# computations/root_digger

Hardware: NVIDIA B200
Metric: root_placements_per_sec (higher is better)
Workload: dtype f64

## Files before the change

### root_digger_b200/csrc/rdk_kernels.cuh

```cuda
#pragma once
#include <cuda_runtime.h>
#include "rdk_lower.hpp"
#include <stdint.h>
#include <type_traits>

namespace rdk {

constexpr int kMaxCats = 32;

__device__ __forceinline__ double dmul(double a, double b) { return __dmul_rn(a, b); }
__device__ __forceinline__ double dadd(double a, double b) { return __dadd_rn(a, b); }
__device__ __forceinline__ double dsub(double a, double b) { return __dsub_rn(a, b); }
__device__ __forceinline__ double ddiv(double a, double b) { return __ddiv_rn(a, b); }
__device__ __forceinline__ double dfma(double a, double b, double c) { return __fma_rn(a, b, c); }

#define RDK_SCALE_THRESHOLD 0x1p-256
#define RDK_SCALE_FACTOR 0x1p+256
#define RDK_LOG_SCALE_THRESHOLD (-177.44567822334599)

static __constant__ double kLogConst[9] = {
    6.93147180369123816490e-01, 1.90821492927058770002e-10,
    6.666666666666735130e-01,   3.999999999940941908e-01,
    2.857142874366239149e-01,   2.222219843214978396e-01,
    1.818357216161805012e-01,   1.531383769920937332e-01,
// ... 53 lines not shown
    }
}

__device__ __forceinline__ double norm1_4(const double* A) {
  double best = 0.0;
#pragma unroll
  for (int j = 0; j < 4; ++j) {
    double s = fabs(A[0 * 4 + j]);
    s = dadd(s, fabs(A[1 * 4 + j]));
    s = dadd(s, fabs(A[2 * 4 + j]));
    s = dadd(s, fabs(A[3 * 4 + j]));
    if (s > best) best = s;
  }
  return best;
}

__device__ inline void solve4(double* M, double* N, double* X) {
  for (int c = 0; c < 4; ++c) {
    int    piv = c;
    double best = fabs(M[c * 4 + c]);
    for (int r = c + 1; r < 4; ++r) {
      double v = fabs(M[r * 4 + c]);
      if (v > best) {
        best = v;
        piv = r;
      }
    }
    if (piv != c) {
      for (int j = 0; j < 4; ++j) {
        double t = M[c * 4 + j];
        M[c * 4 + j] = M[piv * 4 + j];
        M[piv * 4 + j] = t;
        t = N[c * 4 + j];
        N[c * 4 + j] = N[piv * 4 + j];
        N[piv * 4 + j] = t;
      }
    }
    for (int r = c + 1; r < 4; ++r) {
      double f = ddiv(M[r * 4 + c], M[c * 4 + c]);
      for (int j = c + 1; j < 4; ++j) M[r * 4 + j] = dsub(M[r * 4 + j], dmul(f, M[c * 4 + j]));
      for (int j = 0; j < 4; ++j) N[r * 4 + j] = dsub(N[r * 4 + j], dmul(f, N[c * 4 + j]));
    }
  }
  for (int r = 3; r >= 0; --r)
    for (int j = 0; j < 4; ++j) {
      double s = N[r * 4 + j];
      for (int q = r + 1; q < 4; ++q) s = dsub(s, dmul(M[r * 4 + q], X[q * 4 + j]));
      X[r * 4 + j] = ddiv(s, M[r * 4 + r]);
    }
}

__device__ inline void expm4(const double* Ain, double* E) {
  const double TH3 = 1.495585217958292e-2, TH5 = 2.539398330063230e-1,
               TH7 = 9.504178996162932e-1, TH9 = 2.097847961257068e0,
               TH13 = 5.371920351148152e0;
  double A[16], U[16], V[16];
#pragma unroll
  for (int i = 0; i < 16; ++i) A[i] = Ain[i];
  double n1 = norm1_4(A);
  int    s = 0;
  int    deg = 13;
  if (n1 <= TH3)
    deg = 3;
  else if (n1 <= TH5)
    deg = 5;
  else if (n1 <= TH7)
    deg = 7;
  else if (n1 <= TH9)
    deg = 9;
  if (deg == 13) {
    while (n1 > TH13) {
      n1 = dmul(n1, 0.5);
      ++s;
    }
    double sc = __longlong_as_double((long long)(uint64_t)(1023 - s) << 52);
#pragma unroll
    for (int i = 0; i < 16; ++i) A[i] = dmul(A[i], sc);
  }
  double A2[16], A4[16], A6[16];
  mm4(A, A, A2);
  if (deg == 13) {
    const double b0 = 64764752532480000., b1 = 32382376266240000., b2 = 7771770303897600.,
                 b3 = 1187353796428800., b4 = 129060195264000., b5 = 10559470521600.,
                 b6 = 670442572800., b7 = 33522128640., b8 = 1323241920., b9 = 40840800.,
                 b10 = 960960., b11 = 16380., b12 = 182., b13 = 1.;
    double W1[16], Z1[16], W[16], T[16];
    mm4(A2, A2, A4);
    mm4(A4, A2, A6);
#pragma unroll
    for (int i = 0; i < 16; ++i) {
      double t = dmul(b13, A6[i]);
      t = dadd(t, dmul(b11, A4[i]));
      t = dadd(t, dmul(b9, A2[i]));
      W1[i] = t;
      t = dmul(b12, A6[i]);
      t = dadd(t, dmul(b10, A4[i]));
      t = dadd(t, dmul(b8, A2[i]));
      Z1[i] = t;
    }
    mm4(A6, W1, T);
#pragma unroll
    for (int i = 0; i < 16; ++i) {
      double id = (i % 5 == 0) ? 1.0 : 0.0;
      double t = dmul(b7, A6[i]);
      t = dadd(t, dmul(b5, A4[i]));
      t = dadd(t, dmul(b3, A2[i]));
      t = dadd(t, dmul(b1, id));
      W[i] = dadd(T[i], t);
    }
    mm4(A, W, U);
    mm4(A6, Z1, T);
#pragma unroll
    for (int i = 0; i < 16; ++i) {
      double id = (i % 5 == 0) ? 1.0 : 0.0;
      double t = dmul(b6, A6[i]);
      t = dadd(t, dmul(b4, A4[i]));
      t = dadd(t, dmul(b2, A2[i]));
      t = dadd(t, dmul(b0, id));
      V[i] = dadd(T[i], t);
    }
  } else {
    double A8[16], W[16];
    if (deg >= 5) mm4(A2, A2, A4);
    if (deg >= 7) mm4(A4, A2, A6);
    if (deg >= 9) mm4(A6, A2, A8);
    for (int i = 0; i < 16; ++i) {
      double id = (i % 5 == 0) ? 1.0 : 0.0;
      double w, v;
      if (deg == 3) {
        w = dmul(1., A2[i]);
        v = dmul(12., A2[i]);
        W[i] = dadd(w, dmul(60., id));
        V[i] = dadd(v, dmul(120., id));
      } else if (deg == 5) {
        w = dmul(1., A4[i]);
        w = dadd(w, dmul(420., A2[i]));
        v = dmul(30., A4[i]);
        v = dadd(v, dmul(3360., A2[i]));
        W[i] = dadd(w, dmul(15120., id));
        V[i] = dadd(v, dmul(30240., id));
      } else if (deg == 7) {
        w = dmul(1., A6[i]);
        w = dadd(w, dmul(1512., A4[i]));
        w = dadd(w, dmul(277200., A2[i]));
        v = dmul(56., A6[i]);
        v = dadd(v, dmul(25200., A4[i]));
        v = dadd(v, dmul(1995840., A2[i]));
        W[i] = dadd(w, dmul(8648640., id));
        V[i] = dadd(v, dmul(17297280., id));
      } else {
        w = dmul(1., A8[i]);
        w = dadd(w, dmul(3960., A6[i]));
        w = dadd(w, dmul(2162160., A4[i]));
        w = dadd(w, dmul(302702400., A2[i]));
        v = dmul(90., A8[i]);
        v = dadd(v, dmul(110880., A6[i]));
        v = dadd(v, dmul(30270240., A4[i]));
        v = dadd(v, dmul(2075673600., A2[i]));
        W[i] = dadd(w, dmul(8821612800., id));
        V[i] = dadd(v, dmul(17643225600., id));
      }
    }
    mm4(A, W, U);
  }
  double M[16], N[16];
#pragma unroll
  for (int i = 0; i < 16; ++i) {
    M[i] = dsub(V[i], U[i]);
    N[i] = dadd(V[i], U[i]);
  }
  solve4(M, N, E);
  for (int q = 0; q < s; ++q) {
    double T[16];
    mm4(E, E, T);
#pragma unroll
    for (int i = 0; i < 16; ++i) E[i] = T[i];
  }
}

__device__ inline void build_q_nonrev(const double* r, const double* pi, double* Q) {
  int k = 0;
  for (int i = 0; i < 4; ++i)
    for (int j = 0; j < 4; ++j)
      if (i != j) Q[i * 4 + j] = dmul(r[k++], pi[j]);
  for (int i = 0; i < 4; ++i) {
    double s = 0.0;
    bool   first = true;
    for (int j = 0; j < 4; ++j) {
      if (j == i) continue;
      if (first) {
        s = Q[i * 4 + j];
        first = false;
      } else
        s = dadd(s, Q[i * 4 + j]);
    }
    Q[i * 4 + i] = -s;
  }
  double mu = dmul(pi[0], -Q[0]);
  mu = dadd(mu, dmul(pi[1], -Q[5]));
  mu = dadd(mu, dmul(pi[2], -Q[10]));
  mu = dadd(mu, dmul(pi[3], -Q[15]));
  for (int i = 0; i < 16; ++i) Q[i] = ddiv(Q[i], mu);
}

__host__ __device__ __forceinline__ unsigned tip_mask_of_code(unsigned code) {
  return (unsigned)((0x0FEDCBA976538421ULL >> (4 * code)) & 15ULL);
}
__host__ __device__ __forceinline__ unsigned tip_code_of_mask(unsigned mask) {
  return (unsigned)((0xEDCBA9837652410FULL >> (4 * mask)) & 15ULL);
}

constexpr int kPTabDoubles = 18;
constexpr int kTipTabDoubles = 64;
constexpr int kTabDoubles = 64;
constexpr int kSlotDoubles = kPTabDoubles + kTipTabDoubles;

struct PmatEntry {
  unsigned slot;
  unsigned pad;
  double   t;
};

constexpr int kPmatInline = 16;
struct PmatArgs {
  const PmatEntry* entries;
  int              n;
  int              K;
  double           r[12];
  double           pi[4];
  double           pinv;
  double           rates[kMaxCats];
  double*          pool;
  PmatEntry        inl[kPmatInline];
};

#ifndef RDK_PROGRAM_KERNEL_ONLY
__global__ void __launch_bounds__(64) pmat_expm_nonrev_kernel(const __grid_constant__ PmatArgs a) {
  int tid = blockIdx.x * blockDim.x + threadIdx.x;
  if (tid >= a.n * a.K) return;
  int       e = tid / a.K, k = tid - e * a.K;
  PmatEntry ent = (a.n <= kPmatInline) ? a.inl[e] : a.entries[e];
  double    Q[16], A[16], E[16];
  double    r[12], pi[4];
  for (int i = 0; i < 12; ++i) r[i] = a.r[i];
  for (int i = 0; i < 4; ++i) pi[i] = a.pi[i];
  build_q_nonrev(r, pi, Q);
  double c = ddiv(dmul(a.rates[k], ent.t), dsub(1.0, a.pinv));
  for (int i = 0; i < 16; ++i) A[i] = dmul(Q[i], c);
  expm4(A, E);
  double* slot = a.pool + (size_t)ent.slot * a.K * kSlotDoubles;
  double* out = slot + (size_t)k * kPTabDoubles;
  for (int i = 0; i < 16; ++i) out[i] = E[i];
  out[16] = out[17] = 0.0;
  double* tab = slot + (size_t)a.K * kPTabDoubles;
  for (int i = 0; i < 4; ++i)
    for (unsigned code = 0; code < 16; ++code) {
      unsigned m = tip_mask_of_code(code);
      double   x = dmul(E[i * 4 + 0], (m & 1u) ? 1.0 : 0.0);
      x = dadd(x, dmul(E[i * 4 + 1], (m & 2u) ? 1.0 : 0.0));
      x = dadd(x, dmul(E[i * 4 + 2], (m & 4u) ? 1.0 : 0.0));
      x = dadd(x, dmul(E[i * 4 + 3], (m & 8u) ? 1.0 : 0.0));
      tab[((size_t)code * a.K + k) * 4 + i] = x;
    }
}

#endif

struct alignas(16) Instr {
  double*              parent;
  const void*          c1;
  const void*          c2;
  unsigned*            pscale;
  const unsigned*      c1scale;
  const unsigned*      c2scale;
  const double*        P1;
  const double*        P2;
  unsigned             flags;
  unsigned             slot;
  unsigned             pad[2];
};
static_assert(sizeof(Instr) == 80, "Instr layout");

constexpr int kProgInline = 8;
constexpr int kMaxChunks = 16;
struct ProgArgs {
  const Instr*    prog;
  int             n_instr;
  unsigned        nelem;
  unsigned        n_witer;
  unsigned        it0;
  const unsigned* weights;
  double*         partials;
  unsigned        partial_stride;
  double*         persite;
  unsigned        persite_unweighted;
  double          pi[4];
  double          w[kMaxCats];
  unsigned        n_chunks;
  unsigned        chunk_off[kMaxChunks + 1];
  Instr           inl[kProgInline];
  size_t          row_stride;
};

template <int K>
struct Ring {
  static constexpr int      kDepth = K <= 8 ? 8 : (K == 16 ? 4 : 2);
  static constexpr int      kLogDepth = kDepth == 8 ? 3 : (kDepth == 4 ? 2 : 1);
  static constexpr unsigned kTabBytes = kTabDoubles * K * 8;
  static constexpr unsigned kPBytes = kPTabDoubles * K * 8;
  static constexpr unsigned kInstrBytes = 128;
  static constexpr unsigned kSlotBytes = kInstrBytes + 2 * kTabBytes;
  static constexpr unsigned kSmemBytes = kDepth * kSlotBytes + 2 * kDepth * 8;
};

struct d4 {
  double v[4];
};

__device__ __forceinline__ d4 ld_clv(const void* base, unsigned e) {
  const char* q = reinterpret_cast<const char*>(base) + (size_t)e * 32u;
  d4          r;
  asm volatile("ld.global.cg.v4.f64 {%0,%1,%2,%3}, [%4];\n"
               : "=d"(r.v[0]), "=d"(r.v[1]), "=d"(r.v[2]), "=d"(r.v[3])
               : "l"(q));
  return r;
}
__device__ __forceinline__ void st_clv(double* base, unsigned e, const d4& x) {
  char* q = reinterpret_cast<char*>(base) + (size_t)e * 32u;
  asm volatile("st.global.cg.v4.f64 [%0], {%1,%2,%3,%4};\n" ::"l"(q), "d"(x.v[0]), "d"(x.v[1]), "d"(x.v[2]),
               "d"(x.v[3])
               : "memory");
}

__device__ __forceinline__ unsigned smem_u32(const void* p) { return (unsigned)__cvta_generic_to_shared(p); }
__device__ __forceinline__ void mbar_init(unsigned long long* bar, unsigned count) {
  asm volatile("mbarrier.init.shared::cta.b64 [%0], %1;\n" ::"r"(smem_u32(bar)), "r"(count) : "memory");
}
__device__ __forceinline__ void mbar_expect_tx(unsigned long long* bar, unsigned bytes) {
  asm volatile("mbarrier.arrive.expect_tx.shared::cta.b64 _, [%0], %1;\n" ::"r"(smem_u32(bar)), "r"(bytes)
               : "memory");
}
__device__ __forceinline__ void mbar_arrive(unsigned long long* bar) {
  asm volatile("mbarrier.arrive.shared::cta.b64 _, [%0];\n" ::"r"(smem_u32(bar)) : "memory");
}
__device__ __forceinline__ void mbar_wait(unsigned long long* bar, unsigned parity) {
  asm volatile(
      "{\n"
      ".reg .pred P1;\n"
      "LAB_WAIT:\n"
      "mbarrier.try_wait.parity.shared::cta.b64 P1, [%0], %1;\n"
      "@P1 bra DONE;\n"
      "bra LAB_WAIT;\n"
      "DONE:\n"
      "}\n" ::"r"(smem_u32(bar)),
      "r"(parity)
      : "memory");
}
__device__ __forceinline__ bool mbar_try_wait(unsigned long long* bar, unsigned parity) {
  unsigned ok;
  asm volatile(
      "{\n"
      ".reg .pred P1;\n"
      "mbarrier.try_wait.parity.shared::cta.b64 P1, [%1], %2;\n"
      "selp.u32 %0, 1, 0, P1;\n"
      "}\n"
      : "=r"(ok)
      : "r"(smem_u32(bar)), "r"(parity)
      : "memory");
  return ok != 0;
}
__device__ __forceinline__ void bulk_g2s(void* dst, const void* src, unsigned bytes, unsigned long long* bar) {
  asm volatile("cp.async.bulk.shared::cluster.global.mbarrier::complete_tx::bytes [%0], [%1], %2, [%3];\n" ::"r"(
                   smem_u32(dst)),
               "l"(src), "r"(bytes), "r"(smem_u32(bar))
               : "memory");
}

__device__ __forceinline__ int hi_word(double x) { return __double2hiint(x); }
constexpr int kScaleThresholdHi = (1023 - 256) << 20;

constexpr unsigned kProducerSleepNs = 200;

template <int K, int E, int MAXT, int MINB, bool ROWS = false>
__global__ void __launch_bounds__(MAXT, MINB) clv_program_kernel(const __grid_constant__ ProgArgs a) {
  static_assert(32 % K == 0, "K must divide the warp size");
  using R = Ring<K>;
  constexpr unsigned D = R::kDepth;
  extern __shared__ __align__(128) unsigned char smem_raw[];
  unsigned long long* const s_full = reinterpret_cast<unsigned long long*>(smem_raw + D * R::kSlotBytes);
  unsigned long long* const s_empty = s_full + D;

  const unsigned tid = threadIdx.x;
  unsigned       lane;
  asm volatile("mov.u32 %0, %%laneid;\n" : "=r"(lane));
  const unsigned wib = tid >> 5;
  const unsigned n_cons = (blockDim.x >> 5) - 1u;

  const Instr* prog = a.prog;
  unsigned     n_instr = (unsigned)a.n_instr;
  const bool   inline_prog = a.prog == nullptr;
  if (a.n_chunks > 1) {
    prog += a.chunk_off[blockIdx.y];
    n_instr = a.chunk_off[blockIdx.y + 1] - a.chunk_off[blockIdx.y];
  }

  const unsigned c_begin = a.it0 + (unsigned)(((unsigned long long)a.n_witer * blockIdx.x) / gridDim.x);
  const unsigned c_end = a.it0 + (unsigned)(((unsigned long long)a.n_witer * (blockIdx.x + 1)) / gridDim.x);
  const unsigned c_len = c_end - c_begin;
  const unsigned passes = ((c_len + n_cons - 1) / n_cons + E - 1) / E;
  const unsigned total = passes * n_instr;

  if (tid == 0) {
#pragma unroll
    for (unsigned s = 0; s < D; ++s) {
      mbar_init(&s_full[s], 1);
      mbar_init(&s_empty[s], n_cons);
    }
    asm volatile("fence.mbarrier_init.release.cluster;\n" ::: "memory");
  }
  __syncthreads();

  if (wib == n_cons) {
    for (unsigned base = 0; base < total; base += 32u) {
      const unsigned j = base + lane;
      int4           w0 = make_int4(0, 0, 0, 0), w1 = w0, w2 = w0, w3 = w0, w4 = w0;
      if (j < total) {
        const unsigned idx = j % n_instr;
        const int4*    src = reinterpret_cast<const int4*>(inline_prog ? &a.inl[idx] : &prog[idx]);
        w0 = src[0];
        w1 = src[1];
        w2 = src[2];
        w3 = src[3];
        w4 = src[4];
      }
      const unsigned cnt = min(32u, total - base);
      for (unsigned t = 0; t < cnt; ++t) {
        if (lane == t) {
          const unsigned s = j & (D - 1u);
          while (!mbar_try_wait(&s_empty[s], ((j >> R::kLogDepth) & 1u) ^ 1u)) __nanosleep(kProducerSleepNs);
          unsigned char* slot = smem_raw + s * R::kSlotBytes;
          int4*          dst = reinterpret_cast<int4*>(slot);
          dst[0] = w0;
          dst[1] = w1;
          dst[2] = w2;
          dst[3] = w3;
          dst[4] = w4;
          const unsigned fl = (unsigned)w4.x;
          unsigned       b1 = 0, b2 = 0;
          if (!(fl & (fLoadV | fNop))) {
            b1 = (fl & fTip1) ? R::kTabBytes : R::kPBytes;
            b2 = (fl & fTip2) ? R::kTabBytes : R::kPBytes;
          }
          mbar_expect_tx(&s_full[s], b1 + b2);
          if (b1) {
            const unsigned long long p1 = ((unsigned long long)(unsigned)w3.y << 32) | (unsigned)w3.x;
            bulk_g2s(slot + R::kInstrBytes, reinterpret_cast<const void*>(p1), b1, &s_full[s]);
          }
          if (b2) {
            const unsigned long long p2 = ((unsigned long long)(unsigned)w3.w << 32) | (unsigned)w3.z;
            bulk_g2s(slot + R::kInstrBytes + R::kTabBytes, reinterpret_cast<const void*>(p2), b2, &s_full[s]);
          }
        }
        __syncwarp();
      }
    }
    return;
  }

  constexpr unsigned SPW = 32 / K;
  const unsigned     k = lane % K;
  const unsigned     sl = lane / K;
  const unsigned     lane0 = lane - k;
  unsigned           gmask = 0;
#pragma unroll
  for (int j = 0; j < K; ++j) gmask |= 1u << (j + lane0);

  const unsigned it_begin = c_begin + (unsigned)(((unsigned long long)c_len * wib) / n_cons);
  const unsigned it_end = c_begin + (unsigned)(((unsigned long long)c_len * (wib + 1)) / n_cons);
  const unsigned last_site = a.nelem / K - 1;

  auto slot_of = [&](unsigned j) -> const unsigned char* { return smem_raw + (j & (D - 1u)) * R::kSlotBytes; };
  auto wait_full = [&](unsigned j) { mbar_wait(&s_full[j & (D - 1u)], (j >> R::kLogDepth) & 1u); };
  auto release = [&](unsigned j) {
    __syncwarp();
    if (lane == 0) mbar_arrive(&s_empty[j & (D - 1u)]);
  };

  d4       v[E];
  unsigned vcnt[E];
  d4       c1r[E];
  unsigned m1[E], m2n[E], cnt1[E];
#pragma unroll
  for (int u = 0; u < E; ++u) {
#pragma unroll
    for (int i = 0; i < 4; ++i) v[u].v[i] = c1r[u].v[i] = 0.0;
    vcnt[u] = cnt1[u] = 0;
    m1[u] = m2n[u] = 15u;
  }

  unsigned jg = 0;
  for (unsigned pass = 0; pass < passes; ++pass) {
    if (!(it_begin + pass * E < it_end)) {
      for (unsigned ii = 0; ii < n_instr; ++ii, ++jg) {
        wait_full(jg);
        release(jg);
      }
      continue;
    }
    unsigned it[E], e[E], site[E], wgt[E];
#pragma unroll
    for (int u = 0; u < E; ++u) {
      const unsigned i0 = it_begin + pass * E + u;
      it[u] = i0 < it_end ? i0 : it_end - 1;
      unsigned st = it[u] * SPW + sl;
      if (st > last_site) st = last_site;
      site[u] = st;
      e[u] = st * K + k;
      wgt[u] = __ldg(a.weights + st);
    }

    auto load_operands = [&](const Instr& in) __attribute__((always_inline)) {
      const unsigned fl = in.flags;
      if (fl & fTip1) {
        const unsigned char* t = reinterpret_cast<const unsigned char*>(in.c1);
#pragma unroll
        for (int u = 0; u < E; ++u) m1[u] = __ldg(t + site[u]);
      } else if (!(fl & fNop)) {
        const void* g = in.c1;
#pragma unroll
        for (int u = 0; u < E; ++u) c1r[u] = ld_clv(g, e[u]);
      }
      if (fl & fTip2) {
        const unsigned char* t = reinterpret_cast<const unsigned char*>(in.c2);
#pragma unroll
        for (int u = 0; u < E; ++u) m2n[u] = __ldg(t + site[u]);
      }
#pragma unroll
      for (int u = 0; u < E; ++u) cnt1[u] = 0;
      if (fl & fCnt1) {
        const unsigned* s1 = in.c1scale;
#pragma unroll
        for (int u = 0; u < E; ++u) cnt1[u] = __ldcg(s1 + site[u]);
      }
    };

    auto load_v = [&](const Instr& in) __attribute__((always_inline)) {
      const unsigned fl = in.flags;
      if (fl & fLoadV2) {
        const void* g = in.c2;
#pragma unroll
        for (int u = 0; u < E; ++u) v[u] = ld_clv(g, e[u]);
#pragma unroll
        for (int u = 0; u < E; ++u) vcnt[u] = 0;
        if (fl & fCnt2M) {
          const unsigned* s2 = in.c2scale;
#pragma unroll
          for (int u = 0; u < E; ++u) vcnt[u] = __ldcg(s2 + site[u]);
        }
      }
    };

    auto rescale = [&](d4(&r)[E], unsigned(&cnt)[E]) __attribute__((always_inline)) {
      int mx[E], mn = 0x7fffffff;
#pragma unroll
      for (int u = 0; u < E; ++u) {
        mx[u] = max(max(hi_word(r[u].v[0]), hi_word(r[u].v[1])), max(hi_word(r[u].v[2]), hi_word(r[u].v[3])));
        mn = min(mn, mx[u]);
      }
      if (!__any_sync(0xffffffffu, mn < kScaleThresholdHi)) return;
      unsigned m[E], any = 0;
#pragma unroll
      for (int u = 0; u < E; ++u) {
        m[u] = __ballot_sync(0xffffffffu, mx[u] < kScaleThresholdHi);
        unsigned t = m[u];
#pragma unroll
        for (int sft = 1; sft < K; sft <<= 1) t &= t >> sft;
        any |= t;
      }
      constexpr unsigned kSiteBase = K == 1 ? 0xffffffffu : (K == 2 ? 0x55555555u : (K == 4 ? 0x11111111u : (K == 8 ? 0x01010101u : (K == 16 ? 0x00010001u : 1u))));
      if (any & kSiteBase) {
#pragma unroll
        for (int u = 0; u < E; ++u) {
          if ((m[u] & gmask) == gmask) {
#pragma unroll
            for (int i = 0; i < 4; ++i) r[u].v[i] = dmul(r[u].v[i], RDK_SCALE_FACTOR);
            cnt[u] += 1;
          }
        }
      }
    };

    auto evaluate = [&](const Instr& in, const unsigned fl, const d4(&r)[E], const unsigned(&cnt)[E])
                        __attribute__((always_inline)) {
      double term[E];
#pragma unroll
      for (int u = 0; u < E; ++u) {
        double t = dmul(a.pi[0], r[u].v[0]);
        t = dfma(a.pi[1], r[u].v[1], t);
        t = dfma(a.pi[2], r[u].v[2], t);
        t = dfma(a.pi[3], r[u].v[3], t);
        double tm = dmul(a.w[0], __shfl_sync(0xffffffffu, t, lane0));
#pragma unroll
        for (int kk = 1; kk < K; ++kk) {
          double tk = __shfl_sync(0xffffffffu, t, lane0 + kk);
          tm = dfma(a.w[kk], tk, tm);
        }
        term[u] = tm;
      }
      const unsigned eslot = in.slot;
      if constexpr (E <= K) {
        double   x = term[0];
        unsigned cn = cnt[0], st = site[0], iw = it[0], wg = wgt[0];
#pragma unroll
        for (int u = 1; u < E; ++u)
          if (k == (unsigned)u) {
            x = term[u];
            cn = cnt[u];
            st = site[u];
            iw = it[u];
            wg = wgt[u];
          }
        double l = 0.0;
        if (k < (unsigned)E && iw * SPW + sl <= last_site) {
          l = rd_log(x);
          if (fl & fEvalScaler) l = dadd(l, dmul((double)cn, RDK_LOG_SCALE_THRESHOLD));
          const double lw = dmul(l, (double)wg);
          if constexpr (ROWS) a.persite[(size_t)eslot * a.row_stride + st] = l;
          else if (a.persite && eslot == 0) a.persite[st] = a.persite_unweighted ? l : lw;
          l = lw;
        }
#pragma unroll
        for (int off2 = 1; off2 < (int)SPW; off2 <<= 1) l = dadd(l, __shfl_xor_sync(0xffffffffu, l, off2 * K));
        if (sl == 0 && k < (unsigned)E) a.partials[(size_t)eslot * a.partial_stride + iw] = l;
      } else {
#pragma unroll
        for (int u = 0; u < E; ++u) {
          double l = 0.0;
          if (k == 0 && it[u] * SPW + sl <= last_site) {
            l = rd_log(term[u]);
            if (fl & fEvalScaler) l = dadd(l, dmul((double)cnt[u], RDK_LOG_SCALE_THRESHOLD));
            const double lw = dmul(l, (double)wgt[u]);
            if constexpr (ROWS) a.persite[(size_t)eslot * a.row_stride + site[u]] = l;
            else if (a.persite && eslot == 0) a.persite[site[u]] = a.persite_unweighted ? l : lw;
            l = lw;
          }
#pragma unroll
          for (int off2 = 1; off2 < (int)SPW; off2 <<= 1) l = dadd(l, __shfl_xor_sync(0xffffffffu, l, off2 * K));
          if (lane == 0) a.partials[(size_t)eslot * a.partial_stride + it[u]] = l;
        }
      }
    };

    wait_full(jg);
    load_operands(*reinterpret_cast<const Instr*>(slot_of(jg)));
    load_v(*reinterpret_cast<const Instr*>(slot_of(jg)));

    for (unsigned ii = 0; ii < n_instr; ++ii, ++jg) {
      const unsigned char* slot = slot_of(jg);
      const Instr&         in = *reinterpret_cast<const Instr*>(slot);
      const unsigned       fl = in.flags;
      const unsigned char* tab1 = slot + R::kInstrBytes;
      const unsigned char* tab2 = tab1 + R::kTabBytes;
      const bool           main_op = !(fl & (fLoadV | fNop));

      d4       y[E];
      unsigned cnt[E];
      unsigned m2c[E];
#pragma unroll
      for (int u = 0; u < E; ++u) {
        m2c[u] = m2n[u];
        cnt[u] = cnt1[u] + ((fl & fCnt2V) ? vcnt[u] : 0u);
      }

      if (main_op) {
        if (fl & fTip1) {
#pragma unroll
          for (int u = 0; u < E; ++u) {
            const double2* t = reinterpret_cast<const double2*>(tab1 + (m1[u] * K + k) * 32u);
            const double2  lo = t[0], hi = t[1];
            y[u].v[0] = lo.x;
            y[u].v[1] = lo.y;
            y[u].v[2] = hi.x;
            y[u].v[3] = hi.y;
          }
        } else {
          const double2* p = reinterpret_cast<const double2*>(tab1 + k * (kPTabDoubles * 8));
#pragma unroll
          for (int i = 0; i < 4; ++i) {
            const double2 p01 = p[i * 2], p23 = p[i * 2 + 1];
#pragma unroll
            for (int u = 0; u < E; ++u) {
              double s = dmul(p01.x, c1r[u].v[0]);
              s = dfma(p01.y, c1r[u].v[1], s);
              s = dfma(p23.x, c1r[u].v[2], s);
              s = dfma(p23.y, c1r[u].v[3], s);
              y[u].v[i] = s;
            }
          }
        }
      } else if (fl & fLoadV) {
#pragma unroll
        for (int u = 0; u < E; ++u) {
          v[u] = c1r[u];
          vcnt[u] = cnt1[u];
        }
      }

      if (ii + 1 < n_instr) {
        wait_full(jg + 1);
        load_operands(*reinterpret_cast<const Instr*>(slot_of(jg + 1)));
      }

      const bool keep_v = (fl & fEval) != 0;
      if (main_op) {
        if (fl & fTip2) {
#pragma unroll
          for (int u = 0; u < E; ++u) {
            const double2* t = reinterpret_cast<const double2*>(tab2 + (m2c[u] * K + k) * 32u);
            const double2  lo = t[0], hi = t[1];
            y[u].v[0] = dmul(y[u].v[0], lo.x);
            y[u].v[1] = dmul(y[u].v[1], lo.y);
            y[u].v[2] = dmul(y[u].v[2], hi.x);
            y[u].v[3] = dmul(y[u].v[3], hi.y);
          }
        } else {
          const double2* p = reinterpret_cast<const double2*>(tab2 + k * (kPTabDoubles * 8));
#pragma unroll
          for (int i = 0; i < 4; ++i) {
            const double2 p01 = p[i * 2], p23 = p[i * 2 + 1];
#pragma unroll
            for (int u = 0; u < E; ++u) {
              double s = dmul(p01.x, v[u].v[0]);
              s = dfma(p01.y, v[u].v[1], s);
              s = dfma(p23.x, v[u].v[2], s);
              s = dfma(p23.y, v[u].v[3], s);
              y[u].v[i] = dmul(y[u].v[i], s);
            }
          }
        }
      }

      if (main_op) {
        if (fl & fScale) rescale(y, cnt);
        if (keep_v) {
          evaluate(in, fl, y, cnt);
        } else {
          if (fl & fWrite) {
            double* par = in.parent;
#pragma unroll
            for (int u = 0; u < E; ++u) st_clv(par, e[u], y[u]);
          }
          if ((fl & fWriteS) && k == 0) {
            unsigned* ps = in.pscale;
#pragma unroll
            for (int u = 0; u < E; ++u) __stcg(ps + site[u], cnt[u]);
          }
#pragma unroll
          for (int u = 0; u < E; ++u) {
            v[u] = y[u];
            vcnt[u] = cnt[u];
          }
        }
      }
      if (fl & fEvalV) evaluate(in, fl, v, vcnt);
      if (ii + 1 < n_instr) load_v(*reinterpret_cast<const Instr*>(slot_of(jg + 1)));
      release(jg);
    }
  }
}

template <int K>
cudaError_t launch_program(const ProgArgs& a, int grid, int threads, int E, bool rows, cudaStream_t st);
template <> cudaError_t launch_program<1>(const ProgArgs&, int, int, int, bool, cudaStream_t);
template <> cudaError_t launch_program<2>(const ProgArgs&, int, int, int, bool, cudaStream_t);
template <> cudaError_t launch_program<4>(const ProgArgs&, int, int, int, bool, cudaStream_t);
template <> cudaError_t launch_program<8>(const ProgArgs&, int, int, int, bool, cudaStream_t);
template <> cudaError_t launch_program<16>(const ProgArgs&, int, int, int, bool, cudaStream_t);
template <> cudaError_t launch_program<32>(const ProgArgs&, int, int, int, bool, cudaStream_t);
struct LaunchShape {
  int threads, ctas_per_sm;
};
constexpr LaunchShape launch_shape(int E) {
  return E == 4 ? LaunchShape{384, 1} : (E == 3 ? LaunchShape{512, 1} : (E == 2 ? LaunchShape{320, 2} : LaunchShape{512, 2}));
}

#ifndef RDK_PROGRAM_KERNEL_ONLY
__global__ void __launch_bounds__(256) tree_reduce_kernel(const double* __restrict__ in,
                                                           unsigned in_stride, unsigned n_in,
                                                           unsigned span, unsigned n_nodes,
                                                           double* __restrict__ out,
                                                           unsigned out_stride, unsigned out_offset) {
  __shared__ double sm[256];
  const unsigned R = span < 256u ? span : 256u;
  const unsigned L = span / R;
  const unsigned slot = blockIdx.y, t = threadIdx.x;
  const unsigned b = blockIdx.x * (256u / R) + t / R;
  const unsigned tr = t % R;
  const double*  p = in + (size_t)slot * in_stride;
  double         res = 0.0;
  if (b < n_nodes) {
    const unsigned long long base = (unsigned long long)b * span + (unsigned long long)tr * L;
    if (base < n_in) {
      double st[32];
      int    top = 0;
      for (unsigned i = 0; i < L; ++i) {
        unsigned long long idx = base + i;
        double             s = idx < n_in ? p[idx] : 0.0;
        for (unsigned j = i; j & 1u; j >>= 1) s = dadd(st[--top], s);
        st[top++] = s;
      }
      res = st[0];
    }
  }
  sm[t] = res;
  __syncthreads();
  for (unsigned w = 1; w < R; w <<= 1) {
    if ((tr % (2 * w)) == 0) sm[t] = dadd(sm[t], sm[t + w]);
    __syncthreads();
  }
  if (tr == 0 && b < n_nodes) out[(size_t)slot * out_stride + out_offset + b] = sm[0 + t];
}

__global__ void __launch_bounds__(256) tip_hist_kernel(const unsigned char* __restrict__ tips,
                                                        size_t tip_stride, unsigned ntips,
                                                        unsigned sites,
                                                        const unsigned* __restrict__ weights,
                                                        unsigned long long* __restrict__ hist) {
  __shared__ unsigned long long sh[16];
  if (threadIdx.x < 16) sh[threadIdx.x] = 0;
  __syncthreads();
  unsigned long long local[16];
#pragma unroll
  for (int i = 0; i < 16; ++i) local[i] = 0;
  const size_t total = (size_t)ntips * sites;
  for (size_t idx = (size_t)blockIdx.x * blockDim.x + threadIdx.x; idx < total;
       idx += (size_t)gridDim.x * blockDim.x) {
    unsigned tip = (unsigned)(idx / sites), s = (unsigned)(idx - (size_t)tip * sites);
    unsigned m = tip_mask_of_code(tips[(size_t)tip * tip_stride + s] & 15u);
    unsigned w = weights[s];
#pragma unroll
    for (int i = 0; i < 16; ++i)
      if (m == (unsigned)i) local[i] += w;
  }
#pragma unroll
  for (int i = 0; i < 16; ++i)
    if (local[i]) atomicAdd(&sh[i], local[i]);
  __syncthreads();
  if (threadIdx.x < 16 && sh[threadIdx.x]) atomicAdd(&hist[threadIdx.x], sh[threadIdx.x]);
}

__global__ void tip_expand_kernel(const unsigned char* __restrict__ tip, unsigned sites, int K,
                                  double* __restrict__ out) {
  size_t e = (size_t)blockIdx.x * blockDim.x + threadIdx.x;
  if (e >= (size_t)sites * K) return;
  unsigned m = tip_mask_of_code(tip[e / K] & 15u);
  for (int j = 0; j < 4; ++j) out[e * 4 + j] = ((m >> j) & 1u) ? 1.0 : 0.0;
}

#endif

}
```

### root_digger_b200/csrc/rdk_lower.hpp

```cpp
#pragma once
#include <algorithm>
#include <cstdint>
#include <utility>
#include <vector>

namespace rdk {

enum : unsigned {
  rWrite = 1u,
  rEval = 2u,
  rLoadOnly = 4u,
};
constexpr unsigned kNoClv = 0xffffffffu;

struct ROp {
  unsigned parent;
  int      pscale;
  unsigned c1, c2;
  int      c1scale, c2scale;
  unsigned pm1, pm2;
  unsigned flags;
  unsigned slot;
  unsigned id;
};

enum : unsigned {
  fTip1 = 1u,
  fTip2 = 2u,
  fWrite = 4u,
  fWriteS = 8u,
  fEval = 16u,
  fScale = 32u,
  fLoadV = 64u,
  fNop = 128u,
  fEvalV = 256u,
  fCnt1 = 512u,
  fCnt2V = 1024u,
  fEvalScaler = 2048u,
  fLoadV2 = 4096u,
  fCnt2M = 8192u,
};

struct LInstr {
  unsigned flags;
  unsigned parent;
  int      pscale;
  unsigned c1;
  int      c1scale;
  unsigned c2;
  int      c2scale;
  unsigned pm1, pm2;
  unsigned slot;
  unsigned src;
  bool     swapped;
};

constexpr unsigned kNoSrc = 0xffffffffu;

struct LowerOptions {
  unsigned tips = 0;
  bool                     discard_writes = false;
  const std::vector<char> *scratch_clv = nullptr;
  const std::vector<char> *scratch_scaler = nullptr;
};

struct LowerStats {
  unsigned loadv = 0;
  unsigned stores_dropped = 0;
  unsigned forwarded = 0;
};

inline void lower_program(const std::vector<ROp> &ops, const std::vector<unsigned> &chunk_off,
                          const LowerOptions &opt, std::vector<LInstr> &out,
                          std::vector<unsigned> &out_chunk_off, LowerStats *stats = nullptr) {
  out.clear();
  out_chunk_off.clear();
  LowerStats        st;
  const unsigned    tips = opt.tips;
  std::vector<unsigned> bounds = chunk_off;
  if (bounds.size() < 2) bounds = {0u, (unsigned)ops.size()};
  auto is_tip = [&](unsigned c) { return c < tips; };

  for (size_t ch = 0; ch + 1 < bounds.size(); ++ch) {
    out_chunk_off.push_back((unsigned)out.size());
    const size_t chunk_first = out.size();
    unsigned     vptr = kNoClv;
    int          vscale = -1;
    auto guard_raw = [&](unsigned clv, int scaler) {
      if (out.size() == chunk_first) return;
      const LInstr &pv = out.back();
      const bool    hazard = ((pv.flags & fWrite) && pv.parent == clv) ||
                          ((pv.flags & fWriteS) && scaler >= 0 && pv.pscale == scaler);
      if (!hazard) return;
      LInstr nop{};
      nop.src = kNoSrc;
      nop.flags = fNop;
      nop.parent = kNoClv;
      nop.pscale = -1;
      nop.c1 = kNoClv;
      nop.c1scale = -1;
      nop.c2 = kNoClv;
      nop.c2scale = -1;
      out.push_back(nop);
    };
    for (unsigned i = bounds[ch]; i < bounds[ch + 1]; ++i) {
      const ROp &op = ops[i];
      LInstr     li{};
      li.parent = kNoClv;
      li.pscale = -1;
      li.c2 = kNoClv;
      li.c1scale = li.c2scale = -1;
      li.slot = op.slot;
      li.src = kNoSrc;
      if (op.flags & rLoadOnly) {
        const bool in_v = vptr == op.c1 && vscale == op.c1scale;
        if (in_v) {
          li.flags = fNop | fEvalV;
          li.c1 = kNoClv;
          ++st.forwarded;
        } else {
          guard_raw(op.c1, op.c1scale);
          li.flags = fLoadV | fEvalV | (op.c1scale >= 0 ? fCnt1 : 0u);
          li.c1 = op.c1;
          li.c1scale = op.c1scale;
          vptr = op.c1;
          vscale = op.c1scale;
        }
        if (op.c1scale >= 0) li.flags |= fEvalScaler;
        out.push_back(li);
        continue;
      }
      unsigned c1 = op.c1, c2 = op.c2, pm1 = op.pm1, pm2 = op.pm2;
      int      s1 = op.c1scale, s2 = op.c2scale;
      bool swapped = false;
      auto swap_children = [&]() {
        std::swap(c1, c2);
        std::swap(pm1, pm2);
        std::swap(s1, s2);
        swapped = !swapped;
      };
      unsigned fl = 0;
      bool     load_v = false;
      if (is_tip(c1) && is_tip(c2)) {
        fl |= fTip1 | fTip2;
        if (s2 >= 0 && s1 < 0) swap_children();
        s2 = -1;
      } else if (is_tip(c1) || is_tip(c2)) {
        if (is_tip(c2)) swap_children();
        fl |= fTip1;
        if (!(vptr == c2 && vscale == s2)) load_v = true;
        else ++st.forwarded;
      } else {
        if (vptr == c2 && vscale == s2) {
          ++st.forwarded;
        } else if (vptr == c1 && vscale == s1) {
          swap_children();
          ++st.forwarded;
        } else {
          load_v = true;
        }
      }
      if (load_v) {
        fl |= fLoadV2 | (s2 >= 0 ? fCnt2M : 0u);
        ++st.loadv;
      }
      if (s1 >= 0) fl |= fCnt1;
      if (!(fl & fTip2) && s2 >= 0) fl |= fCnt2V;
      if (op.pscale >= 0) fl |= fScale;
      li.c1 = c1;
      li.c1scale = s1;
      li.c2 = (fl & (fTip2 | fLoadV2)) ? c2 : kNoClv;
      li.c2scale = (fl & fCnt2M) ? s2 : -1;
      li.pm1 = pm1;
      li.pm2 = pm2;
      li.src = op.id;
      li.swapped = swapped;
      if ((op.flags & rEval) && !(op.flags & rWrite)) {
        fl |= fEval;
        if (fl & fScale) fl |= fEvalScaler;
      } else {
        if (op.flags & rWrite) {
          fl |= fWrite;
          li.parent = op.parent;
          if (op.pscale >= 0) {
            fl |= fWriteS;
            li.pscale = op.pscale;
          }
        }
        if (op.flags & rEval) {
          fl |= fEvalV;
          if (fl & fScale) fl |= fEvalScaler;
        }
        vptr = op.parent;
        vscale = op.pscale;
      }
      li.flags = fl;
      guard_raw((fl & fTip1) ? kNoClv : li.c1, li.c1scale);
      out.push_back(li);
    }

    unsigned max_clv = 0, max_sc = 0;
    for (size_t j = chunk_first; j < out.size(); ++j) {
      const LInstr &x = out[j];
      if (x.parent != kNoClv) max_clv = std::max(max_clv, x.parent + 1);
      if (x.c1 != kNoClv) max_clv = std::max(max_clv, x.c1 + 1);
      if (x.c2 != kNoClv) max_clv = std::max(max_clv, x.c2 + 1);
      if (x.c2scale >= 0) max_sc = std::max(max_sc, (unsigned)x.c2scale + 1);
      if (x.pscale >= 0) max_sc = std::max(max_sc, (unsigned)x.pscale + 1);
      if (x.c1scale >= 0) max_sc = std::max(max_sc, (unsigned)x.c1scale + 1);
    }
    auto out_needed_clv = [&](unsigned c) {
      if (opt.discard_writes) return false;
      if (opt.scratch_clv && c < opt.scratch_clv->size() && (*opt.scratch_clv)[c]) return false;
      return true;
    };
    auto out_needed_sc = [&](unsigned s) {
      if (opt.discard_writes) return false;
      if (opt.scratch_scaler && s < opt.scratch_scaler->size() && (*opt.scratch_scaler)[s]) return false;
      return true;
    };
    std::vector<char> live_clv(max_clv), live_sc(max_sc);
    for (unsigned c = 0; c < max_clv; ++c) live_clv[c] = out_needed_clv(c) ? 1 : 0;
    for (unsigned s = 0; s < max_sc; ++s) live_sc[s] = out_needed_sc(s) ? 1 : 0;
    for (size_t j = out.size(); j-- > chunk_first;) {
      LInstr &x = out[j];
      if (x.flags & fWrite) {
        if (!live_clv[x.parent]) {
          x.flags &= ~fWrite;
          ++st.stores_dropped;
        }
        live_clv[x.parent] = 0;
      }
      if (x.flags & fWriteS) {
        if (!live_sc[x.pscale]) x.flags &= ~fWriteS;
        live_sc[x.pscale] = 0;
      }
      const bool loads_c1 = !(x.flags & (fTip1 | fNop));
      if (loads_c1 && x.c1 != kNoClv) live_clv[x.c1] = 1;
      if ((x.flags & fCnt1) && x.c1scale >= 0) live_sc[x.c1scale] = 1;
      if (x.flags & fLoadV2) live_clv[x.c2] = 1;
      if (x.flags & fCnt2M) live_sc[x.c2scale] = 1;
    }
  }
  out_chunk_off.push_back((unsigned)out.size());
  if (stats) *stats = st;
}

struct ForestInfo {
  std::vector<int>      consumer;
  std::vector<unsigned> weight;
  std::vector<char>     joins;
};

inline bool analyse_forest(const std::vector<ROp> &ops, unsigned tips, ForestInfo &f) {
  const size_t n = ops.size();
  unsigned     max_clv = tips;
  int          max_sc = 0;
  for (const ROp &r : ops) {
    if (r.parent != kNoClv) max_clv = std::max(max_clv, r.parent + 1);
    if (r.c1 != kNoClv) max_clv = std::max(max_clv, r.c1 + 1);
    if (r.c2 != kNoClv) max_clv = std::max(max_clv, r.c2 + 1);
    max_sc = std::max(max_sc, std::max(r.pscale, std::max(r.c1scale, r.c2scale)) + 1);
  }
  std::vector<int>  wclv(max_clv, -1), wsc((size_t)max_sc, -1);
  std::vector<char> xclv(max_clv, 0), xsc((size_t)max_sc, 0);
  f.consumer.assign(n, -1);
  f.weight.assign(n, 1u);
  f.joins.assign(n, 0);
  for (size_t i = 0; i < n; ++i) {
    const ROp &r = ops[i];
    auto       read = [&](unsigned c, int s) -> bool {
      int prod = -1;
      if (c != kNoClv && c >= tips) {
        prod = wclv[c];
        if (prod < 0) {
          xclv[c] = 1;
        } else {
          if (f.consumer[prod] != -1) return false;
          f.consumer[prod] = (int)i;
          f.weight[i] += f.weight[prod];
          if (f.joins[prod]) f.joins[i] = 1;
        }
      }
      if (s >= 0) {
        if (wsc[s] < 0)
          xsc[s] = 1;
        else if (wsc[s] != prod)
          return false;
      }
      return true;
    };
    if (!read(r.c1, r.c1scale)) return false;
    if (!(r.flags & rLoadOnly) && !read(r.c2, r.c2scale)) return false;
    if ((r.flags & (rEval | rLoadOnly)) || !(r.flags & rWrite)) f.joins[i] = 1;
    if (r.flags & rWrite) {
      if (r.parent == kNoClv || r.parent < tips) return false;
      if (wclv[r.parent] >= 0 || xclv[r.parent]) return false;
      wclv[r.parent] = (int)i;
      if (r.pscale >= 0) {
        if (wsc[r.pscale] >= 0 || xsc[r.pscale]) return false;
        wsc[r.pscale] = (int)i;
      }
    }
  }
  return true;
}

inline unsigned assign_subtree_groups(const ForestInfo &f, unsigned n_groups, unsigned cap, std::vector<int> &group,
                                      unsigned &longest, unsigned &n_join) {
  const size_t n = f.consumer.size();
  group.assign(n, -1);
  std::vector<int>                           unit(n, -1);
  std::vector<std::pair<unsigned, unsigned>> units;
  n_join = 0;
  for (size_t i = n; i-- > 0;) {
    const int c = f.consumer[i];
    if (c >= 0 && unit[c] >= 0) {
      unit[i] = unit[c];
    } else if (!f.joins[i] && f.weight[i] <= cap) {
      unit[i] = (int)units.size();
      units.emplace_back(f.weight[i], (unsigned)units.size());
    } else {
      ++n_join;
    }
  }
  longest = 0;
  if (units.size() < 2 || n_groups < 2) return 0;
  std::sort(units.begin(), units.end(), [](const std::pair<unsigned, unsigned> &a, const std::pair<unsigned, unsigned> &b) {
    return a.first != b.first ? a.first > b.first : a.second < b.second;
  });
  const unsigned        g_used = (unsigned)std::min<size_t>(n_groups, units.size());
  std::vector<unsigned> load(g_used, 0u), of_unit(units.size(), 0u);
  for (const auto &u : units) {
    unsigned best = 0;
    for (unsigned g = 1; g < g_used; ++g)
      if (load[g] < load[best]) best = g;
    load[best] += u.first;
    of_unit[u.second] = best;
  }
  for (unsigned g = 0; g < g_used; ++g) longest = std::max(longest, load[g]);
  for (size_t i = 0; i < n; ++i)
    if (unit[i] >= 0) group[i] = (int)of_unit[unit[i]];
  return g_used;
}

inline void split_by_group(const std::vector<ROp> &ops, const std::vector<int> &group, unsigned g_used,
                           std::vector<ROp> &grouped, std::vector<unsigned> &group_off, std::vector<ROp> &join) {
  group_off.assign(g_used + 1, 0u);
  for (size_t i = 0; i < ops.size(); ++i)
    if (group[i] >= 0) ++group_off[(size_t)group[i] + 1];
  for (unsigned g = 0; g < g_used; ++g) group_off[g + 1] += group_off[g];
  grouped.resize(group_off[g_used]);
  join.clear();
  std::vector<unsigned> at(group_off.begin(), group_off.end() - 1);
  for (size_t i = 0; i < ops.size(); ++i) {
    if (group[i] >= 0)
      grouped[at[(size_t)group[i]]++] = ops[i];
    else
      join.push_back(ops[i]);
  }
}

inline void lower_grouped(const std::vector<ROp> &grouped, const std::vector<unsigned> &group_off,
                          const std::vector<ROp> &join, const LowerOptions &opt, std::vector<LInstr> &out_groups,
                          std::vector<unsigned> &out_group_off, std::vector<LInstr> &out_join, LowerStats *stats) {
  LowerOptions      gopt = opt;
  std::vector<char> scr_clv, scr_sc;
  if (opt.discard_writes) {
    unsigned max_clv = 0;
    int      max_sc = 0;
    for (const ROp &r : grouped) {
      if (r.parent != kNoClv) max_clv = std::max(max_clv, r.parent + 1);
      max_sc = std::max(max_sc, r.pscale + 1);
    }
    scr_clv.assign(max_clv, 1);
    scr_sc.assign((size_t)max_sc, 1);
    auto needed = [&](unsigned c, int sc) {
      if (c != kNoClv && c < scr_clv.size()) scr_clv[c] = 0;
      if (sc >= 0 && (size_t)sc < scr_sc.size()) scr_sc[(size_t)sc] = 0;
    };
    for (const ROp &r : join) {
      needed(r.c1, r.c1scale);
      if (!(r.flags & rLoadOnly)) needed(r.c2, r.c2scale);
    }
    gopt.discard_writes = false;
    gopt.scratch_clv = &scr_clv;
    gopt.scratch_scaler = &scr_sc;
  }
  LowerStats a, b;
  lower_program(grouped, group_off, gopt, out_groups, out_group_off, &a);
  std::vector<unsigned> none;
  lower_program(join, std::vector<unsigned>(), opt, out_join, none, &b);
  if (stats) {
    stats->loadv = a.loadv + b.loadv;
    stats->stores_dropped = a.stores_dropped + b.stores_dropped;
    stats->forwarded = a.forwarded + b.forwarded;
  }
}

}
```

### root_digger_b200/csrc/rdk_program_inst.cu

```cuda
#define RDK_PROGRAM_KERNEL_ONLY 1
#include "rdk_kernels.cuh"

#ifndef RDK_INST_K
#error "compile with -DRDK_INST_K=<rate categories>"
#endif

namespace rdk {
namespace {

template <int K, int E, bool ROWS>
cudaError_t launch_inst(const ProgArgs &a, int grid, int threads, cudaStream_t st) {
  constexpr LaunchShape shape = launch_shape(E);
  const size_t          smem = Ring<K>::kSmemBytes;
  static bool           configured = false;
  if (!configured) {
    cudaError_t err = cudaFuncSetAttribute(clv_program_kernel<K, E, shape.threads, shape.ctas_per_sm, ROWS>,
                                           cudaFuncAttributeMaxDynamicSharedMemorySize, (int)smem);
    if (err != cudaSuccess) return err;
    configured = true;
  }
  if (threads > shape.threads) threads = shape.threads;
  clv_program_kernel<K, E, shape.threads, shape.ctas_per_sm, ROWS>
      <<<dim3((unsigned)grid, a.n_chunks > 1 ? a.n_chunks : 1u), threads, smem, st>>>(a);
  return cudaSuccess;
}

template <bool ROWS>
cudaError_t launch_e(const ProgArgs &a, int grid, int threads, int E, cudaStream_t st) {
  constexpr int K = RDK_INST_K;
  switch (E) {
    case 1: return launch_inst<K, 1, ROWS>(a, grid, threads, st);
    case 2: return launch_inst<K, 2, ROWS>(a, grid, threads, st);
    case 3: return launch_inst<K, 3, ROWS>(a, grid, threads, st);
    default: return launch_inst<K, 4, ROWS>(a, grid, threads, st);
  }
}

}

template <>
cudaError_t launch_program<RDK_INST_K>(const ProgArgs &a, int grid, int threads, int E, bool rows, cudaStream_t st) {
  return rows ? launch_e<true>(a, grid, threads, E, st) : launch_e<false>(a, grid, threads, E, st);
}

}
```

Before: 125,900.

## Stage CLV and scaler operand tiles into shared memory via bulk async copies

For E==4 and K<=8, the producer warp now bulk-copies each pass's contiguous tile of child CLVs and scaler counts into the ring slot alongside the P-tables. Consumers read those operands from shared memory instead of issuing per-thread global loads. Work is reassigned so a CTA tile is contiguous across warps. The lowering pass marks operands written by the immediately preceding instruction as direct, and those are still loaded from global memory. A proxy fence after writes orders them against later bulk copies, and the ring depth drops to 2 with much larger slots, which may reduce prefetch depth and occupancy.

Result: slower. 84510, median of 6 (-32.9%).

```diff
diff --git a/root_digger_b200/csrc/rdk_kernels.cuh b/root_digger_b200/csrc/rdk_kernels.cuh
--- a/root_digger_b200/csrc/rdk_kernels.cuh
+++ b/root_digger_b200/csrc/rdk_kernels.cuh
@@ -379,15 +379,23 @@
   size_t          row_stride;
 };
 
-template <int K>
+__host__ __device__ constexpr bool stage_operands(int K, int E) { return E == 4 && K <= 8; }
+
+template <int K, bool STAGE>
 struct Ring {
-  static constexpr int      kDepth = K <= 8 ? 8 : (K == 16 ? 4 : 2);
+  static constexpr int      kDepth = STAGE ? (int)kOperandDepth : (K <= 8 ? 8 : (K == 16 ? 4 : 2));
   static constexpr int      kLogDepth = kDepth == 8 ? 3 : (kDepth == 4 ? 2 : 1);
+  static_assert(kDepth == 1 << kLogDepth, "ring depth: a power of two");
   static constexpr unsigned kTabBytes = kTabDoubles * K * 8;
   static constexpr unsigned kPBytes = kPTabDoubles * K * 8;
   static constexpr unsigned kInstrBytes = 128;
-  static constexpr unsigned kSlotBytes = kInstrBytes + 2 * kTabBytes;
-  static constexpr unsigned kSmemBytes = kDepth * kSlotBytes + 2 * kDepth * 8;
+  static constexpr unsigned kTabSlotBytes = kInstrBytes + 2 * kTabBytes;
+  __host__ __device__ static constexpr unsigned clv_tile_bytes(unsigned tile) { return tile * 1024u; }
+  __host__ __device__ static constexpr unsigned sc_run_bytes(unsigned tile) { return tile * (128u / K); }
+  __host__ __device__ static constexpr unsigned slot_bytes(unsigned tile) {
+    return kTabSlotBytes + (STAGE ? 2 * (clv_tile_bytes(tile) + sc_run_bytes(tile)) : 0u);
+  }
+  __host__ __device__ static constexpr unsigned smem_bytes(unsigned tile) { return kDepth * slot_bytes(tile) + 2 * kDepth * 8; }
 };
 
 struct d4 {
@@ -401,6 +409,11 @@
                : "=d"(r.v[0]), "=d"(r.v[1]), "=d"(r.v[2]), "=d"(r.v[3])
                : "l"(q));
   return r;
+}
+__device__ __forceinline__ d4 lds_clv(const unsigned char* tile, unsigned e) {
+  const double2* q = reinterpret_cast<const double2*>(tile + (size_t)e * 32u);
+  const double2  lo = q[0], hi = q[1];
+  return d4{{lo.x, lo.y, hi.x, hi.y}};
 }
 __device__ __forceinline__ void st_clv(double* base, unsigned e, const d4& x) {
   char* q = reinterpret_cast<char*>(base) + (size_t)e * 32u;
@@ -461,17 +474,22 @@
 template <int K, int E, int MAXT, int MINB, bool ROWS = false>
 __global__ void __launch_bounds__(MAXT, MINB) clv_program_kernel(const __grid_constant__ ProgArgs a) {
   static_assert(32 % K == 0, "K must divide the warp size");
-  using R = Ring<K>;
+  constexpr bool STAGE = stage_operands(K, E);
+  using R = Ring<K, STAGE>;
   constexpr unsigned D = R::kDepth;
-  extern __shared__ __align__(128) unsigned char smem_raw[];
-  unsigned long long* const s_full = reinterpret_cast<unsigned long long*>(smem_raw + D * R::kSlotBytes);
-  unsigned long long* const s_empty = s_full + D;
+  constexpr unsigned SPW = 32 / K;
 
   const unsigned tid = threadIdx.x;
   unsigned       lane;
   asm volatile("mov.u32 %0, %%laneid;\n" : "=r"(lane));
   const unsigned wib = tid >> 5;
   const unsigned n_cons = (blockDim.x >> 5) - 1u;
+  const unsigned tile = E * n_cons;
+
+  extern __shared__ __align__(128) unsigned char smem_raw[];
+  const unsigned            slot_bytes = R::slot_bytes(tile);
+  unsigned long long* const s_full = reinterpret_cast<unsigned long long*>(smem_raw + D * slot_bytes);
+  unsigned long long* const s_empty = s_full + D;
 
   const Instr* prog = a.prog;
   unsigned     n_instr = (unsigned)a.n_instr;
@@ -484,8 +502,9 @@
   const unsigned c_begin = a.it0 + (unsigned)(((unsigned long long)a.n_witer * blockIdx.x) / gridDim.x);
   const unsigned c_end = a.it0 + (unsigned)(((unsigned long long)a.n_witer * (blockIdx.x + 1)) / gridDim.x);
   const unsigned c_len = c_end - c_begin;
-  const unsigned passes = ((c_len + n_cons - 1) / n_cons + E - 1) / E;
+  const unsigned passes = (c_len + tile - 1) / tile;
   const unsigned total = passes * n_instr;
+  const unsigned n_sites = a.nelem / K;
 
   if (tid == 0) {
 #pragma unroll
@@ -515,7 +534,7 @@
         if (lane == t) {
           const unsigned s = j & (D - 1u);
           while (!mbar_try_wait(&s_empty[s], ((j >> R::kLogDepth) & 1u) ^ 1u)) __nanosleep(kProducerSleepNs);
-          unsigned char* slot = smem_raw + s * R::kSlotBytes;
+          unsigned char* slot = smem_raw + s * slot_bytes;
           int4*          dst = reinterpret_cast<int4*>(slot);
           dst[0] = w0;
           dst[1] = w1;
@@ -528,7 +547,20 @@
             b1 = (fl & fTip1) ? R::kTabBytes : R::kPBytes;
             b2 = (fl & fTip2) ? R::kTabBytes : R::kPBytes;
           }
-          mbar_expect_tx(&s_full[s], b1 + b2);
+          unsigned c1b = 0, c2b = 0, s1b = 0, s2b = 0, tb = 0;
+          if constexpr (STAGE) {
+            tb = c_begin + (j / n_instr) * tile;
+            const unsigned te = min(tb + tile, c_end);
+            const unsigned clv = (min(te * 32u, a.nelem) - tb * 32u) * 32u;
+            const unsigned run = ((min(te * SPW, n_sites) - tb * SPW) * 4u + 15u) & ~15u;
+            if (!(fl & (fTip1 | fNop | fDirect1))) c1b = clv;
+            if ((fl & fCnt1) && !(fl & fDirect1)) s1b = run;
+            if ((fl & fLoadV2) && !(fl & fDirect2)) {
+              c2b = clv;
+              if (fl & fCnt2M) s2b = run;
+            }
+          }
+          mbar_expect_tx(&s_full[s], b1 + b2 + c1b + c2b + s1b + s2b);
           if (b1) {
             const unsigned long long p1 = ((unsigned long long)(unsigned)w3.y << 32) | (unsigned)w3.x;
             bulk_g2s(slot + R::kInstrBytes, reinterpret_cast<const void*>(p1), b1, &s_full[s]);
@@ -537,6 +569,17 @@
             const unsigned long long p2 = ((unsigned long long)(unsigned)w3.w << 32) | (unsigned)w3.z;
             bulk_g2s(slot + R::kInstrBytes + R::kTabBytes, reinterpret_cast<const void*>(p2), b2, &s_full[s]);
           }
+          if constexpr (STAGE) {
+            auto ptr = [](int lo, int hi) {
+              return reinterpret_cast<const char*>(((unsigned long long)(unsigned)hi << 32) | (unsigned)lo);
+            };
+            unsigned char* const op = slot + R::kTabSlotBytes;
+            const unsigned       ct = R::clv_tile_bytes(tile), st = R::sc_run_bytes(tile);
+            if (c1b) bulk_g2s(op, ptr(w0.z, w0.w) + (size_t)tb * 1024u, c1b, &s_full[s]);
+            if (c2b) bulk_g2s(op + ct, ptr(w1.x, w1.y) + (size_t)tb * 1024u, c2b, &s_full[s]);
+            if (s1b) bulk_g2s(op + 2 * ct, ptr(w2.x, w2.y) + (size_t)tb * SPW * 4u, s1b, &s_full[s]);
+            if (s2b) bulk_g2s(op + 2 * ct + st, ptr(w2.z, w2.w) + (size_t)tb * SPW * 4u, s2b, &s_full[s]);
+          }
         }
         __syncwarp();
       }
@@ -544,7 +587,6 @@
     return;
   }
 
-  constexpr unsigned SPW = 32 / K;
   const unsigned     k = lane % K;
   const unsigned     sl = lane / K;
   const unsigned     lane0 = lane - k;
@@ -552,11 +594,9 @@
 #pragma unroll
   for (int j = 0; j < K; ++j) gmask |= 1u << (j + lane0);
 
-  const unsigned it_begin = c_begin + (unsigned)(((unsigned long long)c_len * wib) / n_cons);
-  const unsigned it_end = c_begin + (unsigned)(((unsigned long long)c_len * (wib + 1)) / n_cons);
-  const unsigned last_site = a.nelem / K - 1;
-
-  auto slot_of = [&](unsigned j) -> const unsigned char* { return smem_raw + (j & (D - 1u)) * R::kSlotBytes; };
+  const unsigned last_site = n_sites - 1;
+
+  auto slot_of = [&](unsigned j) -> const unsigned char* { return smem_raw + (j & (D - 1u)) * slot_bytes; };
   auto wait_full = [&](unsigned j) { mbar_wait(&s_full[j & (D - 1u)], (j >> R::kLogDepth) & 1u); };
   auto release = [&](unsigned j) {
     __syncwarp();
@@ -576,19 +616,20 @@
   }
 
   unsigned jg = 0;
-  for (unsigned pass = 0; pass < passes; ++pass) {
-    if (!(it_begin + pass * E < it_end)) {
+  for (unsigned tb = c_begin; tb < c_end; tb += tile) {
+    const unsigned wb = tb + wib * E;
+    if (!(wb < c_end)) {
       for (unsigned ii = 0; ii < n_instr; ++ii, ++jg) {
         wait_full(jg);
         release(jg);
       }
       continue;
     }
-    unsigned it[E], e[E], site[E], wgt[E];
+    const unsigned wl = min(wb + E, c_end) - 1u;
+    unsigned       it[E], e[E], site[E], wgt[E];
 #pragma unroll
     for (int u = 0; u < E; ++u) {
-      const unsigned i0 = it_begin + pass * E + u;
-      it[u] = i0 < it_end ? i0 : it_end - 1;
+      it[u] = min(wb + u, wl);
       unsigned st = it[u] * SPW + sl;
       if (st > last_site) st = last_site;
       site[u] = st;
@@ -602,7 +643,7 @@
         const unsigned char* t = reinterpret_cast<const unsigned char*>(in.c1);
 #pragma unroll
         for (int u = 0; u < E; ++u) m1[u] = __ldg(t + site[u]);
-      } else if (!(fl & fNop)) {
+      } else if (!STAGE && !(fl & fNop)) {
         const void* g = in.c1;
 #pragma unroll
         for (int u = 0; u < E; ++u) c1r[u] = ld_clv(g, e[u]);
@@ -612,12 +653,39 @@
 #pragma unroll
         for (int u = 0; u < E; ++u) m2n[u] = __ldg(t + site[u]);
       }
-#pragma unroll
-      for (int u = 0; u < E; ++u) cnt1[u] = 0;
-      if (fl & fCnt1) {
-        const unsigned* s1 = in.c1scale;
-#pragma unroll
-        for (int u = 0; u < E; ++u) cnt1[u] = __ldcg(s1 + site[u]);
+      if constexpr (!STAGE) {
+#pragma unroll
+        for (int u = 0; u < E; ++u) cnt1[u] = 0;
+        if (fl & fCnt1) {
+          const unsigned* s1 = in.c1scale;
+#pragma unroll
+          for (int u = 0; u < E; ++u) cnt1[u] = __ldcg(s1 + site[u]);
+        }
+      }
+    };
+
+    auto stage_in = [&](const unsigned char* slot, const Instr& in, d4(&c1s)[E]) __attribute__((always_inline)) {
+      const unsigned       fl = in.flags;
+      const unsigned char* op = slot + R::kTabSlotBytes;
+      const unsigned       ct = R::clv_tile_bytes(tile), st = R::sc_run_bytes(tile);
+      const unsigned       e0 = tb * 32u, s0 = tb * SPW;
+      const bool           d1 = (fl & fDirect1) != 0, d2 = (fl & fDirect2) != 0;
+      if (!(fl & (fTip1 | fNop))) {
+#pragma unroll
+        for (int u = 0; u < E; ++u) c1s[u] = d1 ? ld_clv(in.c1, e[u]) : lds_clv(op, e[u] - e0);
+      }
+#pragma unroll
+      for (int u = 0; u < E; ++u) {
+        const unsigned* s1 = reinterpret_cast<const unsigned*>(op + 2 * ct);
+        cnt1[u] = !(fl & fCnt1) ? 0u : (d1 ? __ldcg(in.c1scale + site[u]) : s1[site[u] - s0]);
+      }
+      if (fl & fLoadV2) {
+#pragma unroll
+        for (int u = 0; u < E; ++u) {
+          const unsigned* s2 = reinterpret_cast<const unsigned*>(op + 2 * ct + st);
+          v[u] = d2 ? ld_clv(in.c2, e[u]) : lds_clv(op + ct, e[u] - e0);
+          vcnt[u] = !(fl & fCnt2M) ? 0u : (d2 ? __ldcg(in.c2scale + site[u]) : s2[site[u] - s0]);
+        }
       }
     };
 
@@ -730,7 +798,7 @@
 
     wait_full(jg);
     load_operands(*reinterpret_cast<const Instr*>(slot_of(jg)));
-    load_v(*reinterpret_cast<const Instr*>(slot_of(jg)));
+    if constexpr (!STAGE) load_v(*reinterpret_cast<const Instr*>(slot_of(jg)));
 
     for (unsigned ii = 0; ii < n_instr; ++ii, ++jg) {
       const unsigned char* slot = slot_of(jg);
@@ -739,6 +807,9 @@
       const unsigned char* tab1 = slot + R::kInstrBytes;
       const unsigned char* tab2 = tab1 + R::kTabBytes;
       const bool           main_op = !(fl & (fLoadV | fNop));
+      d4                   c1s[E];
+      if constexpr (STAGE) stage_in(slot, in, c1s);
+      const d4* const c1 = STAGE ? c1s : c1r;
 
       d4       y[E];
       unsigned cnt[E];
@@ -767,10 +838,10 @@
             const double2 p01 = p[i * 2], p23 = p[i * 2 + 1];
 #pragma unroll
             for (int u = 0; u < E; ++u) {
-              double s = dmul(p01.x, c1r[u].v[0]);
-              s = dfma(p01.y, c1r[u].v[1], s);
-              s = dfma(p23.x, c1r[u].v[2], s);
-              s = dfma(p23.y, c1r[u].v[3], s);
+              double s = dmul(p01.x, c1[u].v[0]);
+              s = dfma(p01.y, c1[u].v[1], s);
+              s = dfma(p23.x, c1[u].v[2], s);
+              s = dfma(p23.y, c1[u].v[3], s);
               y[u].v[i] = s;
             }
           }
@@ -778,7 +849,7 @@
       } else if (fl & fLoadV) {
 #pragma unroll
         for (int u = 0; u < E; ++u) {
-          v[u] = c1r[u];
+          v[u] = c1[u];
           vcnt[u] = cnt1[u];
         }
       }
@@ -840,7 +911,11 @@
         }
       }
       if (fl & fEvalV) evaluate(in, fl, v, vcnt);
-      if (ii + 1 < n_instr) load_v(*reinterpret_cast<const Instr*>(slot_of(jg + 1)));
+      if constexpr (STAGE) {
+        if (fl & (fWrite | fWriteS)) asm volatile("fence.proxy.async.global;\n" ::: "memory");
+      } else if (ii + 1 < n_instr) {
+        load_v(*reinterpret_cast<const Instr*>(slot_of(jg + 1)));
+      }
       release(jg);
     }
   }
diff --git a/root_digger_b200/csrc/rdk_lower.hpp b/root_digger_b200/csrc/rdk_lower.hpp
--- a/root_digger_b200/csrc/rdk_lower.hpp
+++ b/root_digger_b200/csrc/rdk_lower.hpp
@@ -39,7 +39,11 @@
   fEvalScaler = 2048u,
   fLoadV2 = 4096u,
   fCnt2M = 8192u,
-};
+  fDirect1 = 16384u,
+  fDirect2 = 32768u,
+};
+
+constexpr unsigned kOperandDepth = 2;
 
 struct LInstr {
   unsigned flags;
@@ -241,6 +245,18 @@
       if (x.flags & fLoadV2) live_clv[x.c2] = 1;
       if (x.flags & fCnt2M) live_sc[x.c2scale] = 1;
     }
+
+    for (size_t j = chunk_first; j < out.size(); ++j) {
+      LInstr    &x = out[j];
+      const bool c1_clv = !(x.flags & (fTip1 | fNop)), c1_sc = (x.flags & fCnt1) != 0;
+      const bool c2_clv = (x.flags & fLoadV2) != 0, c2_sc = (x.flags & fCnt2M) != 0;
+      for (size_t d = 1; d < kOperandDepth && d <= j - chunk_first; ++d) {
+        const LInstr &w = out[j - d];
+        const bool    wc = (w.flags & fWrite) != 0, ws = (w.flags & fWriteS) != 0;
+        if ((c1_clv && wc && w.parent == x.c1) || (c1_sc && ws && w.pscale == x.c1scale)) x.flags |= fDirect1;
+        if ((c2_clv && wc && w.parent == x.c2) || (c2_sc && ws && w.pscale == x.c2scale)) x.flags |= fDirect2;
+      }
+    }
   }
   out_chunk_off.push_back((unsigned)out.size());
   if (stats) *stats = st;
diff --git a/root_digger_b200/csrc/rdk_program_inst.cu b/root_digger_b200/csrc/rdk_program_inst.cu
--- a/root_digger_b200/csrc/rdk_program_inst.cu
+++ b/root_digger_b200/csrc/rdk_program_inst.cu
@@ -11,15 +11,18 @@
 template <int K, int E, bool ROWS>
 cudaError_t launch_inst(const ProgArgs &a, int grid, int threads, cudaStream_t st) {
   constexpr LaunchShape shape = launch_shape(E);
-  const size_t          smem = Ring<K>::kSmemBytes;
-  static bool           configured = false;
+  using R = Ring<K, stage_operands(K, E)>;
+  constexpr unsigned    kMaxSmem = R::smem_bytes(E * (unsigned)(shape.threads / 32 - 1));
+  static_assert(kMaxSmem <= 227u * 1024u, "the ring must fit the shared memory of one CTA");
+  static bool configured = false;
   if (!configured) {
     cudaError_t err = cudaFuncSetAttribute(clv_program_kernel<K, E, shape.threads, shape.ctas_per_sm, ROWS>,
-                                           cudaFuncAttributeMaxDynamicSharedMemorySize, (int)smem);
+                                           cudaFuncAttributeMaxDynamicSharedMemorySize, (int)kMaxSmem);
     if (err != cudaSuccess) return err;
     configured = true;
   }
   if (threads > shape.threads) threads = shape.threads;
+  const size_t smem = R::smem_bytes(E * (unsigned)(threads / 32 - 1));
   clv_program_kernel<K, E, shape.threads, shape.ctas_per_sm, ROWS>
       <<<dim3((unsigned)grid, a.n_chunks > 1 ? a.n_chunks : 1u), threads, smem, st>>>(a);
   return cudaSuccess;
```
